# Enigmatisms/AdaPT

Hardware: AMD Instinct MI355X
Metric: Msamples/s (W*H*spp/s), unidirectional MIS path tracing (higher is better)
Workload: dtype f32

## Files before the change

adapt_amd/_lib.py:

```python
from __future__ import annotations

import ctypes as C
import os

_HERE = os.path.dirname(os.path.abspath(__file__))
LIB_PATHS = {"fast": os.environ.get("ADAPT_MI_LIB") or os.path.join(_HERE, "libadapt_mi.so"),
             "exact": os.environ.get("ADAPT_MI_LIB_EXACT") or os.path.join(_HERE, "libadapt_mi_exact.so")}
_variant = "exact" if os.environ.get("APT_EXACT", "0") not in ("", "0") else "fast"
LIB_PATH = LIB_PATHS[_variant]

f32p = C.POINTER(C.c_float)
i32p = C.POINTER(C.c_int32)
u32p = C.POINTER(C.c_uint32)
u8p = C.POINTER(C.c_uint8)
f64p = C.POINTER(C.c_double)
APT_N_KERNELS = 5
KERNEL_NAMES = ("generate", "extend", "shade", "shadow", "finalize")


class AptError(RuntimeError):
    pass


class SceneDesc(C.Structure):
# ... 28 lines not shown
    def as_dict(self):
        d = {k: int(getattr(self, k)) for k in ("n_samples", "n_extend", "n_shade", "n_shadow", "n_shadow_traced", "n_lit", "n_draws", "n_poisoned", "n_track")}
        d["launches"] = dict(zip(KERNEL_NAMES, [int(x) for x in self.launches]))
        d["kernel_ms"] = dict(zip(KERNEL_NAMES, [float(x) for x in self.kernel_ms]))
        d["render_ms"] = float(self.render_ms)
        return d


SYMBOLS = {
    "apt_bvh_build": (C.c_int, [f32p, C.c_int32, i32p, C.c_int32, C.POINTER(C.c_void_p)]),
    "apt_bvh_counts": (C.c_int, [C.c_void_p, i32p, i32p, i32p]),
    "apt_bvh_export": (C.c_int, [C.c_void_p, f32p, i32p]),
    "apt_bvh_wide_counts": (C.c_int, [C.c_void_p, i32p, i32p]),
    "apt_flat_records": (C.c_int, [f32p, C.c_int32, i32p, C.c_int32, i32p, f32p, C.c_int32, f32p, C.c_int32, i32p, i32p]),
    "apt_flat_occluders": (C.c_int, [f32p, C.c_int32, i32p, C.c_int32, i32p, f32p, C.c_int32, C.c_int32, i32p, i32p, C.c_int32, f32p, C.c_int32, i32p, i32p]),
    "apt_bvh_wide_export": (C.c_int, [C.c_void_p, u32p, i32p]),
    "apt_bvh_wide_frame": (C.c_int, [C.c_void_p, f32p, f32p]),
    "apt_bvh_free": (None, [C.c_void_p]),
    "apt_bvh_build_linear": (C.c_int, [f32p, C.c_int32, i32p, i32p, C.c_int32, f32p, f32p, C.POINTER(C.c_void_p)]),
    "apt_linear_bvh_counts": (C.c_int, [C.c_void_p, i32p, i32p]),
    "apt_linear_bvh_export": (C.c_int, [C.c_void_p, f32p, f32p, i32p, i32p]),
    "apt_linear_bvh_free": (None, [C.c_void_p]),
    "apt_scene_create": (C.c_int, [C.POINTER(SceneDesc), C.c_int32, C.POINTER(C.c_void_p)]),
    "apt_scene_destroy": (None, [C.c_void_p]),
    "apt_renderer_create": (C.c_int, [C.c_void_p, C.POINTER(RenderCfg), C.POINTER(C.c_void_p)]),
    "apt_renderer_destroy": (None, [C.c_void_p]),
    "apt_render": (C.c_int, [C.c_void_p, C.c_int32]),
    "apt_synchronize": (C.c_int, [C.c_void_p]),
    "apt_tile_shape": (C.c_int, [C.c_void_p, i32p, i32p]),
    "apt_read_pixels": (C.c_int, [C.c_void_p, f32p]),
# ... 71 lines not shown
```

adapt_amd/csrc/api.hip:

```cpp
#include <hip/hip_runtime.h>
#include <chrono>

#include <algorithm>
#include <cmath>
#include <cstdio>
#include <cstdlib>
#include <cstring>
#include <limits>
#include <memory>
#include <string>
#include <vector>

#include "../../include/adapt_mi.h"
#include "bvh_build.hpp"
#include "shade_stage.hpp"
#include "unit_kernels.hpp"
#include "volumetric.hpp"

#define APT_EXPORT extern "C" __attribute__((visibility("default")))

static thread_local std::string g_err;
static int fail(int code, const std::string& msg) { g_err = msg; return code; }
#define HIP_TRY(expr)                                                                              \
    do {                                                                                           \
// ... 95 lines not shown
template <class... V> static bool put(const char* what, DevBuf& b, const V&... v) {
    const hipError_t e = upload(b, v...);
    if (e != hipSuccess) fail(APT_E_HIP, std::string("upload ") + what + ": " + hipGetErrorString(e));
    return e == hipSuccess;
}

struct apt_bvh { apt::BvhData data; apt::BvhData bin3; apt::WideBvhData wide; };

struct apt_scene {
    int device = 0;
    DevScene dev{};
    int bvh_levels = 0;
    DevBuf nodes, prims, slot_prim, normals, vnormals, precom, prim_obj, prim_class, obj_info, emitter_id, bxdf, src, sweep_recs, sweep_tab;
    DevBuf flat_recs, flat_tab, flat_pairs;
    DevBuf flat_occ, flat_occ_tab;
    bool has_flat = false;
    DevBuf uvs, tex_i, tex_f, atlas[3];
    DevBuf prim_shade;
    DevBuf med;
    DevBuf vol_grid;
    bool has_volume = false;
    bool has_null_surface = false;
    std::vector<int> obj_class;
    std::vector<uint8_t> obj_null;
    float box_min[3] = {1e3f, 1e3f, 1e3f}, box_max[3] = {-1e3f, -1e3f, -1e3f};
    int n_classes = 0;
    int class_def[APT_N_CLASS_DEFS] = {};
    int n_prims = 0, n_objects = 0, n_sources = 0, max_obj_prims = 0;
    int bx_mask = 0, src_mask = 0;
    bool has_aabb = false;
// ... 9 lines not shown
    hipEvent_t fin = nullptr;
    LdsPlan plan{};
    Counters* cnt() const { return counters.as<Counters>(); }
};

struct apt_renderer {
    const apt_scene* scene = nullptr;
    apt_render_cfg cfg{};
    Params par{};
    int n_cols = 0, npix = 0, spp_batch = 1;
    int cnt = 0;
    std::vector<Lane> lanes;
    int n_lanes = 1;
    hipStream_t stream() const { return lanes[0].stream; }
    DevBuf accum, scratch, pix_key;
    Counters host_counters{};
    int grid_small = 0, grid_trace = 0, nq = APT_MAX_NQ;
    const ShadeVariant* shade = nullptr;
    int trace_mode = 0;
    int trace_nt = BLOCK;
    int trace_items = BLOCK;
    int sorted = 0;
    int volumetric = 0;
    int dyn_fetch = 0;
    bool tile_ok = false;
    extend_fn extend = nullptr, fix = nullptr;
    int ovf_levels = 0;
    int v_ncls = 0;
    int vev_single = 0;
    vev_shade_fn vev_all = nullptr;
// ... 288 lines not shown
    const int N = s->n_prims;
    if (N > APT_FLAT_MAX_PRIMS || !s->has_sweep || !d->obj_aabb) return APT_OK;
    std::vector<float> fr, ft; int fc[7];
    if (apt::build_flat(d->prims, N, d->obj_info, s->n_objects, prim_class.data(), fr, ft, fc) != 0) return fail(APT_E_INVALID, "apt_scene_create: flat records: obj_info range outside the primitive array");
    if (!put("flat records", s->flat_recs, fr) || !put("flat records", s->flat_tab, ft) || !put("flat record pairs", s->flat_pairs, apt::flat_pairs(fr, fc))) return APT_E_HIP;
    const bool cull = !(getenv("APT_SHADOW_CULL") && atoi(getenv("APT_SHADOW_CULL")) == 0);
    std::vector<float> pts, op; std::vector<int32_t> off, ot; std::vector<uint8_t> keep;
    apt::emitter_points(d->prims, d->obj_info, s->n_objects, d->src_i, d->src_f, s->n_sources, pts, off);
    if (apt::flat_occluders(d->prims, N, fr, ft, fc, pts.data(), off.data(), s->n_sources, cull, op, ot, keep) != 0) return fail(APT_E_INVALID, "apt_scene_create: flat records: bad record");
    if (!put("occluder lists", s->flat_occ, op) || !put("occluder lists", s->flat_occ_tab, ot)) return APT_E_HIP;
    FlatScene& fl = s->dev.flat;
    fl.stream = s->flat_recs.as<float>(); fl.tab = s->flat_tab.as<float4>(); fl.pairs = s->flat_pairs.as<float>();
    fl.occ_pairs = s->flat_occ.as<float>(); fl.occ_tab = s->flat_occ_tab.as<int>();
    fl.defer_all = getenv("APT_FLAT_DEFER_ALL") ? atoi(getenv("APT_FLAT_DEFER_ALL")) : 0;
    fl.n_quads = fc[0]; fl.n_quads_tie = fc[1]; fl.n_gquads = fc[2]; fl.n_gquads_tie = fc[3]; fl.n_tris = fc[4]; fl.n_tris_tie = fc[5]; fl.n_spheres = fc[6];
    s->has_flat = true;
    if (timer.on) fprintf(stderr, "[scene timing] flat records: %d + %d parallelograms, %d + %d convex quads, %d + %d triangles (plain + coplanar groups), %d spheres of %d primitives\n", fc[0], fc[1], fc[2], fc[3], fc[4], fc[5], fc[6], N);
    if (timer.on) for (int e = 0; e < s->n_sources; e++) fprintf(stderr, "[scene timing] occluders of emitter %d: %d parallelograms, %d convex quads, %d triangles, %d spheres\n", e, ot[8 * (size_t)e + 1], ot[8 * (size_t)e + 2], ot[8 * (size_t)e + 3], ot[8 * (size_t)e + 4]);
    timer.tick("flat records");
    return APT_OK;
}
#endif
static int pack_emitters(const apt_scene_desc* d, apt_scene* s) {
    std::vector<DevSrc> sr((size_t)s->n_sources);
    for (int k = 0; k < s->n_sources; k++) {
        const int32_t* si = d->src_i + 4 * k; const float* sf = d->src_f + 11 * k;
        DevSrc& e = sr[(size_t)k]; memset(&e, 0, sizeof(e));
        e.type = si[0]; e.bool_bits = si[1]; e.obj_ref_id = si[2];
        s->src_mask |= 1 << (e.type & 7);
        e.intensity = mk3(sf[0], sf[1], sf[2]); e.dir = mk3(sf[3], sf[4], sf[5]); e.pos = mk3(sf[6], sf[7], sf[8]); e.inv_area = sf[9]; e.r = sf[10];
// ... 224 lines not shown
        for (int g = 0; g < APT_N_GROUPS; g++) { r->group_fn_[g] = kGroupShade[smi][g]; for (int k = 0; k < APT_GROUP_SLOTS; k++) r->group_cls[g][k] = -1; }
        r->shade_name = "sorted, launched in register-footprint groups:";
        for (int g = 0; g < APT_N_GROUPS; g++) r->group_tr_[g] = kGroupShadeTr[smi][g];
        for (int c = 0; c < sc->n_classes; c++) {
            r->group_cls[kClassGroup[sc->class_def[c]]][kClassSlot[sc->class_def[c]]] = c;
            r->shade_name += std::string(c ? "+" : "") + kClassName[sc->class_def[c]];
        }
    } else {
        r->shade_name = r->shade->name;
        if (p.fused == 2) r->shade_name += " [rays traced in place]";
    }
    if (r->transient) r->shade_name += " [transient]";
    if (r->adaptive) r->shade_name += " [adaptive]";
    r->extend = r->dyn_fetch ? kExtendDyn[r->sorted] : (r->trace_mode == 3 ? kExtendFlatHot[r->sorted] : kExtend[r->trace_mode][r->sorted]);
    r->fix = kFixFlat[r->sorted];
    return APT_OK;
}

static int make_lanes(apt_renderer* r) {
    const apt_scene* sc = r->scene;
    const Params& p = r->par;
    const size_t cap = p.cap, sh_subcap = (size_t)p.subcap * (size_t)(p.S > 0 ? p.S : 1), sh_cap = sh_subcap * (size_t)p.nq;
    const int ncls = r->volumetric ? r->v_ncls : (r->sorted ? sc->n_classes : 0);
    if (cap >= ((size_t)1 << 30) || sh_cap >= ((size_t)1 << 30)) { return fail(APT_E_INVALID, "apt_renderer_create: batch too large (queue capacity must stay below 2^30 slots)"); }
    if (p.fused == 2 && cap >= ((size_t)1 << 28)) { return fail(APT_E_INVALID, "apt_renderer_create: batch too large (rays traced in place address 16-byte slots with 32-bit byte offsets: capacity must stay below 2^28)"); }
    if ((size_t)ncls * cap >= ((size_t)1 << 28)) { return fail(APT_E_INVALID, "apt_renderer_create: batch too large (packed class queues address 16-byte slots with 32-bit byte offsets: classes x capacity must stay below 2^28)"); }
    const bool staged = p.fused != 2, tr_uv = !staged && (sc->dev.has_vn || sc->dev.tex_i != nullptr);
    const bool walk_lists = r->volumetric && sc->has_null_surface;
    const size_t l_planes = (size_t)p.l_planes;
    auto carve = [&](float* base, Queues& q) -> size_t {
// ... 205 lines not shown
    if (!std::isfinite(c.adaptive_threshold)) return fail(APT_E_INVALID, "apt_renderer_create: adaptive_threshold must be finite (> 0: adaptive sampling, <= 0: off)");
    if (c.adaptive_threshold > 0.f) {
        if (c.transient_bins > 0)
            return fail(APT_E_INVALID, "apt_renderer_create: adaptive sampling and transient rendering do not combine (transient_bins must be 0 when adaptive_threshold > 0)");
        if (c.adaptive_min_spp <= 0 || c.adaptive_step <= 0)
            return fail(APT_E_INVALID, "apt_renderer_create: adaptive sampling needs adaptive_min_spp > 0 and adaptive_step > 0");
    }
    HIP_TRY(hipSetDevice(c.device));
    apt_renderer* r = new apt_renderer();
    struct Owner { apt_renderer* r; ~Owner() { if (r) apt_renderer_destroy(r); } } owner{r};
    r->scene = sc; r->cfg = c;
    r->adaptive = c.adaptive_threshold > 0.f ? 1 : 0;
    if (int rc = plan_film(r)) return rc;
    pick_traversal(r);
    if (int rc = pick_shading(r)) return rc;
    if (int rc = make_lanes(r)) return rc;
    if (int rc = make_transient(r)) return rc;
    if (int rc = make_adaptive(r)) return rc;
    if (int rc = plan_lds_and_grids(r)) return rc;
    if (int rc = make_overflow_stacks(r)) return rc;
    for (Lane& ln : r->lanes) HIP_TRY(hipStreamSynchronize(ln.stream));
    owner.r = nullptr;
    *out = r;
    return APT_OK;
}

static int grid_for(size_t n, int cap_blocks, int nq, int nt = BLOCK) {
    size_t b = (n + nt - 1) / nt;
    b = ((b + nq - 1) / nq) * nq;
    if (b < (size_t)nq) b = nq;
// ... 156 lines not shown
    hipEvent_t prev_fin = nullptr;
    const int batch_cap = lane_batch(r, n_spp);
    while (done < n_spp) {
        const int B = (n_spp - done < batch_cap) ? (n_spp - done) : batch_cap;
        Lane& ln = r->lanes[(size_t)(batch % r->n_lanes)];
        hipStream_t st = ln.stream;
        const Queues& q = ln.q;
        Counters* cnt = ln.cnt();
        Params p = r->par; p.cnt_base = r->cnt; p.spp_batch = B;
        const size_t total = (size_t)r->npix * (size_t)B;
        if (int rc = begin_batch(r, ln)) return rc;
#if APT_FAST
        if (p.fused == 2) {
            {
                LaunchTimer t(r, 0, st);
                if (r->adaptive) hipLaunchKernelGGL(k_generate_trace_ad, dim3(grid_for(total, r->grid_small, 1)), dim3(BLOCK), 0, st, sc, p, q, cnt, (const uint8_t*)r->aq.active);
                else hipLaunchKernelGGL(k_generate_trace, dim3(grid_for(total, r->grid_small, 1)), dim3(BLOCK), 0, st, sc, p, q, cnt);
            }
            int cur = 0;
            for (int b = 0; b < p.max_bounce; b++) {
                { LaunchTimer t(r, 2, st); hipLaunchKernelGGL(r->shade->traced, dim3(grid_for(total, r->grid_small, nq)), dim3(BLOCK), 0, st, sc, p, q, cnt, cur, b); }
                cur ^= 1;
            }
            if (p.max_bounce > 0) { LaunchTimer t(r, 3, st, false); hipLaunchKernelGGL(r->fix, dim3(r->grid_fix), dim3(BLOCK), 0, st, sc, p, q, cnt, cur, (const uint32_t*)cnt->n_active[cur], ln.plan); }
        } else
#endif
        {
        {
            LaunchTimer t(r, 0, st);
            if (r->adaptive) hipLaunchKernelGGL(k_generate_ad, dim3(grid_for(total, r->grid_small, 1)), dim3(BLOCK), 0, st, p, q, cnt, (const uint8_t*)r->aq.active);
            else hipLaunchKernelGGL(k_generate, dim3(grid_for(total, r->grid_small, 1)), dim3(BLOCK), 0, st, p, q, cnt);
        }
// ... 438 lines not shown
```

adapt_amd/csrc/bvh_build.hpp:

```cpp
#pragma once
#include <algorithm>
#include <cstdint>
#include <cstdlib>
#include <thread>
#include <vector>

#ifndef APT_NODE_BYTES
#define APT_NODE_BYTES 64u
#endif
#define APT_NODE_DWORDS (APT_NODE_BYTES / 4u)
namespace apt {
inline int host_threads() {
    int t = (int)std::thread::hardware_concurrency();
    t = std::max(1, std::min(t, 32));
    if (const char* e = std::getenv("APT_HOST_THREADS")) t = std::max(1, std::atoi(e));
    return t;
}
template <class F>
void parallel_for(int n, int threads, F f) {
    if (threads <= 1 || n < 2048) { for (int i = 0; i < n; i++) f(i); return; }
    const int t = std::min(threads, (n + 511) / 512);
    std::vector<std::thread> pool;
    pool.reserve((size_t)t);
    for (int k = 0; k < t; k++) {
// ... 30 lines not shown
    std::vector<int32_t> node_info;
    int n_nodes() const { return (int)(node_info.size() / 3); }
    int n_prims() const { return (int)(bvh_info.size() / 2); }
};
int build_linear_bvh(const float* prims, int n_prims, const int32_t* obj_prim_cnt, const int32_t* obj_is_sphere, int n_objects,
                     const float world_min[3], const float world_max[3], LinearBvhData& out);

void planar_rows(const float* tri9, float out12[12]);
int build_flat(const float* prims, int n_prims, const int32_t* obj_info, int n_objects, const int32_t* prim_class,
               std::vector<float>& stream, std::vector<float>& tab, int counts[7]);
std::vector<float> flat_pairs(const std::vector<float>& stream, const int counts[7]);
void emitter_points(const float* prims, const int32_t* obj_info, int n_objects, const int32_t* src_i, const float* src_f, int n_sources,
                    std::vector<float>& pts, std::vector<int32_t>& off);
int flat_occluders(const float* prims, int n_prims, const std::vector<float>& stream, const std::vector<float>& tab, const int counts[7],
                   const float* pts, const int32_t* off, int n_emit, bool cull, std::vector<float>& pairs, std::vector<int32_t>& table, std::vector<uint8_t>& keep);
}
```

adapt_amd/csrc/flat_build.cpp:

```cpp
#include <algorithm>
#include <array>
#include <cmath>
#include <cstring>

#include "bvh_build.hpp"

namespace apt {
namespace {
struct D3 { double x, y, z; };
inline D3 sub(D3 a, D3 b) { return {a.x - b.x, a.y - b.y, a.z - b.z}; }
inline D3 add(D3 a, D3 b) { return {a.x + b.x, a.y + b.y, a.z + b.z}; }
inline D3 cross(D3 a, D3 b) { return {a.y * b.z - a.z * b.y, a.z * b.x - a.x * b.z, a.x * b.y - a.y * b.x}; }
inline double dot(D3 a, D3 b) { return a.x * b.x + a.y * b.y + a.z * b.z; }
inline D3 vtx(const float* prims, int k, int v) { const float* p = prims + 9 * (size_t)k + 3 * v; return {p[0], p[1], p[2]}; }

struct Planar { float P0[3], U[4], V[4], T[4]; int prim_a, prim_b; float map_a[6], map_b[6]; bool ok; int obj; bool tie; float lo[3], hi[3]; float far_edges[6]; };

bool make_rows(D3 p0, D3 e1, D3 e2, Planar& r) {
    const D3 n = cross(e1, e2);
    const double det = dot(n, n);
    if (!(det > 0.0) || !std::isfinite(det)) return false;
    const D3 ru = cross(e2, n), rv = cross(n, e1);
    const D3 U = {ru.x / det, ru.y / det, ru.z / det}, V = {rv.x / det, rv.y / det, rv.z / det};
    const double len = std::sqrt(det);
// ... 305 lines not shown
        }
        std::vector<float> st; int c[7] = {0, 0, 0, 0, 0, 0, 0};
        for (int ri = 0; ri < n_rec; ri++) if (kp[ri]) {
            const Rec& r = recs[(size_t)ri];
            st.insert(st.end(), stream.begin() + (long)r.at, stream.begin() + (long)(r.at + (size_t)kRecordFloats[r.sec]));
            c[2 * r.sec]++;
        }
        int32_t* t = table.data() + 8 * (size_t)e;
        t[0] = (int32_t)pairs.size(); t[1] = c[0]; t[2] = c[2]; t[3] = c[4]; t[4] = c[6];
        std::vector<float> pr = flat_pairs(st, c);
        pairs.insert(pairs.end(), pr.begin(), pr.end());
    }
    if (pairs.empty()) pairs.push_back(0.f);
    return 0;
}
}
```

adapt_amd/csrc/stages.hpp:

```cpp
#pragma once
#include <hip/hip_runtime.h>

#include "rng.hpp"
#include "shading.hpp"
#include "traverse.hpp"
#include "vec.hpp"

struct DevMedium {
    int type;
    float ior;
    f3 u_s, u_a, u_e, par, pdf;
};
struct DevVolume {
    int type, xres, yres, zres;
    f3 albedo, trans, mini, maxi, majorant, pdf;
    f3 inv_r0, inv_r1, inv_r2;
    DevMedium ph;
    const float* grid;
};
struct DevScene {
    DevBvh bvh;
    SweepScene sweep;
    FlatScene flat;
    const float* normals;
// ... 253 lines not shown
    SubLoop s;
    s.q = (int)(blockIdx.x % (uint32_t)nq);
    s.first = (blockIdx.x / (uint32_t)nq) * (uint32_t)nt;
    s.stride = (gridDim.x / (uint32_t)nq) * (uint32_t)nt;
    return s;
}
#ifndef APT_TILE_NT
#define APT_TILE_NT 512
#endif
#ifndef APT_TILE_WAVES
#define APT_TILE_WAVES 6
#endif
#define TRACE_NT(MODE) ((MODE) == 2 ? APT_TILE_NT : BLOCK)

template <bool TRACE, bool ADAPTIVE = false>
APT_D void generate_body(const DevScene* sc, const Params& p, const Queues& q, Counters* cnt, const uint8_t* active = nullptr) {
    const uint32_t total = (uint32_t)p.npix * (uint32_t)p.spp_batch;
    const uint32_t n_waves = (total + 63u) / 64u;
    const uint32_t wave_stride = gridDim.x * (BLOCK / 64);
    uint32_t t_samples = 0, t_draws = 0;
    for (uint32_t w = blockIdx.x * (BLOCK / 64) + threadIdx.x / 64u; w < n_waves; w += wave_stride) {
        const uint32_t idx = w * 64u + lane_id();
        const int sq = (int)(w % (uint32_t)p.nq);
        bool valid = idx < total, alive = false;
        f3 dir = mk3(0.f, 0.f, 1.f);
        uint32_t draws = 0;
        if (valid) {
            uint32_t lp = idx % (uint32_t)p.npix, s = idx / (uint32_t)p.npix;
            int i, j; local_to_global(p, lp, i, j);
            for (int pl = 0; pl < p.l_planes; pl++) stL(q.L, p.cap, (idx << 2) | (uint32_t)pl, splat3(0.f));
            alive = !p.do_crop || (i >= p.sx && i < p.ex && j >= p.sy && j < p.ey);
// ... 21 lines not shown
            }
        }
        uint32_t pos;
        uint32_t* q0_counter = &cnt->n_active[0][sq * CNT_PAD];
        if (TRACE) pos = 0;
        else if (p.do_crop || ADAPTIVE) pos = wave_append(alive, q0_counter);
        else {
            pos = (w / (uint32_t)p.nq) * 64u + lane_id();
            unsigned long long m = __ballot(alive);
            if (lane_id() == 0) atomicAdd(q0_counter, (uint32_t)__popcll(m));
        }
#if APT_FAST
        if (TRACE) {
            const f3 cam_o = mk3(p.cam_t[0], p.cam_t[1], p.cam_t[2]);
            float tr_t = 0.f; int tr_run = -1, tr_idx = -1;
            if (__any(alive)) tr_idx = flat_closest1(sc->flat, cam_o, dir, 1e7f, tr_t, tr_run);
            const bool defer = alive && (tr_run >= 0 || flat_needs_cull(sc->flat, dir));
            HitRec hr; hr.t = 1e7f; hr.prim = -1; hr.u = hr.v = 0.f;
            int hit_cls = 0;
            if (alive && !defer && tr_idx >= 0) flat_resolve(sc->flat, tr_idx, tr_t, cam_o, dir, hr, hit_cls);
            const int ocls = !alive ? -1 : (defer ? q.tr_ncls : (hr.prim >= 0 ? (q.tr_ncls > 1 ? hit_cls : 0) : -1));
            const TrAppend app = tr_append_issue(ocls, q.tr_ncls + 1, &cnt->n_tr[0][0][sq * CNT_PAD], APT_MAX_NQ * CNT_PAD);
            pos = tr_append_pos(app, ocls);
            if (alive) t_samples++;
            if (ocls >= 0) {
                const uint32_t slot = (q.tr_stage_top && ocls == q.tr_ncls) ? (uint32_t)sq * p.subcap + p.subcap - 1u - pos : (uint32_t)ocls * p.cap + (uint32_t)sq * p.subcap + pos, so = slot << 4;
                stq(q.tr[0][0], so, make_float4(cam_o.x, cam_o.y, cam_o.z, hr.t));
                stq(q.tr[0][1], so, make_float4(dir.x, dir.y, dir.z, __uint_as_float(tr_pack(hr.prim, draws, false))));
                stq(q.tr[0][2], so, make_float4(1.f, 1.f, 1.f, __uint_as_float(((idx / (uint32_t)p.npix) << p.pix_bits) | (idx % (uint32_t)p.npix))));
                stq(q.tr[0][3], so, make_float4(0.f, 0.f, 0.f, 1.f));
                if (sc->has_vn || sc->tex_i != nullptr) { float2 uv_; uv_.x = hr.u; uv_.y = hr.v; stq(q.tr_uv[0], slot << 3, uv_); }
// ... 8 lines not shown
            stq(q.id[0], so, ((idx / (uint32_t)p.npix) << p.pix_bits) | (idx % (uint32_t)p.npix));
            stq(q.meta[0], so, pack_meta(draws, 0u, false));
            stq(q.pdf[0], so, 1.f);
            t_samples++;
        }
        t_draws += draws;
    }
    const int sq0 = (int)((blockIdx.x * (BLOCK / 64) + threadIdx.x / 64u) % (uint32_t)p.nq);
    flush_stat(t_samples, &cnt->stats[sq0][ST_SAMPLES]);
    if (TRACE) flush_stat(t_samples, &cnt->stats[sq0][ST_EXTEND]);
    flush_stat(t_draws, &cnt->stats[sq0][ST_DRAWS]);
}
__global__ void __launch_bounds__(BLOCK) k_generate(Params p, Queues q, Counters* cnt) { generate_body<false>(nullptr, p, q, cnt); }
__global__ void __launch_bounds__(BLOCK) k_generate_ad(Params p, Queues q, Counters* cnt, const uint8_t* active) { generate_body<false, true>(nullptr, p, q, cnt, active); }
#if APT_FAST
__global__ void __launch_bounds__(BLOCK) k_generate_trace(DevScene sc, Params p, Queues q, Counters* cnt) { generate_body<true>(&sc, p, q, cnt); }
__global__ void __launch_bounds__(BLOCK) k_generate_trace_ad(DevScene sc, Params p, Queues q, Counters* cnt, const uint8_t* active) { generate_body<true, true>(&sc, p, q, cnt, active); }
#endif

template <int MODE, int SORTED>
__global__ void __launch_bounds__(TRACE_NT(MODE), (MODE == 2 ? APT_TILE_WAVES : 1)) k_extend(DevScene sc, Params p, Queues q, Counters* cnt, int cur, const uint32_t* n_src, LdsPlan plan) {
    __shared__ float s_sweep[MODE == 1 ? APT_SWEEP_LDS_FLOATS(BLOCK) : 1];
    const SubLoop sl = sub_loop(p.nq, TRACE_NT(MODE));
    const uint32_t n = n_src[sl.q * CNT_PAD];
    if (cnt && sl.first == 0 && threadIdx.x == 0) {
        cnt->n_shadow[sl.q * CNT_PAD] = 0; cnt->n_active[cur ^ 1][sl.q * CNT_PAD] = 0;
        for (int w = 0; w < 8; w++) cnt->n_walk[w][sl.q * CNT_PAD] = 0;
        cnt->stats[sl.q][ST_EXTEND] += n;
    }
    const float* ro = q.ray_o[cur]; const float* rd = q.ray_d[cur];
    const uint32_t qbase = (uint32_t)sl.q * p.subcap;
    for (uint32_t base = sl.first; base < n; base += sl.stride) {
// ... 582 lines not shown
```

adapt_amd/csrc/traverse.hpp:

```cpp
#pragma once
#include "vec.hpp"

struct DevBvh {
    const uint4* nodes;
    const float4* prims;
    const int* slot_prim;
    int n_nodes, n_prims;
    float gmin[3], ginv[3], gstep[3];
};
#ifndef APT_FAST_LEAVES
#define APT_FAST_LEAVES APT_FAST
#endif
struct HitRec { float t; int prim; float u, v; };

typedef float v2f __attribute__((ext_vector_type(2)));
APT_D v2f sp2(float s) { v2f r; r.x = s; r.y = s; return r; }
APT_D v2f mk2(float a, float b) { v2f r; r.x = a; r.y = b; return r; }

struct WalkRay { f3 o, d, inv, noo; uint32_t octinv4; };
#ifdef APT_WALK_IEEE_RCP
APT_D float walk_rcp(float d) { return (fabsf(d) < 1e-30f) ? copysignf(1e30f, d) : 1.0f / d; }
#else
APT_D float walk_rcp(float d) { return (fabsf(d) < 1e-30f) ? copysignf(1e30f, d) : __builtin_amdgcn_rcpf(d); }
#endif
// ... 698 lines not shown
        occ = occ || flat_blocks(fminf(fminf(u.x, v.x), w.x) >= 0.f, t.x, lim) || flat_blocks(fminf(fminf(u.y, v.y), w.y) >= 0.f, t.y, lim);
    }
    for (int j = 0; j < ns; j++, at += 8) {
        const v2f r2 = ld2c(at + 6);
        const v2f sx = ld2c(at) - ox, sy = ld2c(at + 2) - oy, sz = ld2c(at + 4) - oz;
        const v2f cn2 = (sx * sx + sy * sy) + sz * sz;
        const v2f proj = (dx * sx + dy * sy) + dz * sz;
        const v2f c2ray = cn2 - proj * proj;
        const v2f disc = r2 - c2ray;
        const float cut0 = sqrtf(disc.x), cut1 = sqrtf(disc.y);
        const float ta = proj.x + ((cn2.x > r2.x + 1e-4f) ? -cut0 : cut0), tb = proj.y + ((cn2.y > r2.y + 1e-4f) ? -cut1 : cut1);
        occ = occ || flat_blocks(c2ray.x < r2.x, ta, lim) || flat_blocks(c2ray.y < r2.y, tb, lim);
    }
    return occ;
}
APT_D int flat_closest1(const FlatScene& fl, f3 o, f3 d, float lim, float& t_out, int& runner) {
    cf_ptr at = (cf_ptr)fl.pairs;
    const v2f ox = sp2(o.x), oy = sp2(o.y), oz = sp2(o.z), dx = sp2(d.x), dy = sp2(d.y), dz = sp2(d.z);
    FlatBest b; b.t = lim; b.idx = -1; b.runner = -1;
    auto solve = [&](cf_ptr r, v2f& t, v2f& u, v2f& v) {
        const v2f sx = ox - ld2c(r), sy = oy - ld2c(r + 2), sz = oz - ld2c(r + 4);
        const v2f ux = ld2c(r + 6), uy = ld2c(r + 8), uz = ld2c(r + 10);
        const v2f vx = ld2c(r + 12), vy = ld2c(r + 14), vz = ld2c(r + 16);
        const v2f tx = ld2c(r + 18), ty = ld2c(r + 20), tz = ld2c(r + 22);
        const v2f t_o = fma2(tx, sx, fma2(ty, sy, tz * sz));
        const v2f t_d = fma2(tx, dx, fma2(ty, dy, tz * dz));
        v2f inv; inv.x = __builtin_amdgcn_rcpf(t_d.x); inv.y = __builtin_amdgcn_rcpf(t_d.y);
        t = -t_o * inv;
        const v2f px = fma2(t, dx, sx), py = fma2(t, dy, sy), pz = fma2(t, dz, sz);
        u = fma2(ux, px, fma2(uy, py, uz * pz));
        v = fma2(vx, px, fma2(vy, py, vz * pz));
    };
    int idx = 0;
    {
        const int n = fl.n_quads + fl.n_quads_tie, n_plain = fl.n_quads >> 1;
        int j = 0;
        for (; j < n_plain; j++, idx += 2, at += 24) {
            v2f t, u, v; solve(at, t, u, v);
            const v2f a = u - sp2(0.5f), c = v - sp2(0.5f);
            b = flat_candidate<false>(b, fmaxf(fabsf(a.x), fabsf(c.x)) <= 0.5f, t.x, idx);
            b = flat_candidate<false>(b, fmaxf(fabsf(a.y), fabsf(c.y)) <= 0.5f, t.y, idx + 1);
        }
        for (; 2 * j < n; j++, idx += 2, at += 24) {
            v2f t, u, v; solve(at, t, u, v);
            const v2f a = u - sp2(0.5f), c = v - sp2(0.5f);
            b = flat_candidate<true>(b, fmaxf(fabsf(a.x), fabsf(c.x)) <= 0.5f, t.x, idx);
            b = flat_candidate<true>(b, 2 * j + 1 < n && fmaxf(fabsf(a.y), fabsf(c.y)) <= 0.5f, t.y, idx + 1);
        }
        idx = n;
    }
    {
        const int n = fl.n_gquads + fl.n_gquads_tie, n_plain = fl.n_gquads >> 1, first = idx;
        int j = 0;
        for (; j < n_plain; j++, idx += 2, at += 36) {
            v2f t, u, v; solve(at, t, u, v);
            const v2f e1 = fma2(ld2c(at + 24), u, fma2(ld2c(at + 26), v, ld2c(at + 28))), e2 = fma2(ld2c(at + 30), u, fma2(ld2c(at + 32), v, ld2c(at + 34)));
            b = flat_candidate<false>(b, fminf(fminf(u.x, v.x), fminf(e1.x, e2.x)) >= 0.f, t.x, idx);
            b = flat_candidate<false>(b, fminf(fminf(u.y, v.y), fminf(e1.y, e2.y)) >= 0.f, t.y, idx + 1);
        }
        for (; 2 * j < n; j++, idx += 2, at += 36) {
            v2f t, u, v; solve(at, t, u, v);
            const v2f e1 = fma2(ld2c(at + 24), u, fma2(ld2c(at + 26), v, ld2c(at + 28))), e2 = fma2(ld2c(at + 30), u, fma2(ld2c(at + 32), v, ld2c(at + 34)));
            b = flat_candidate<true>(b, fminf(fminf(u.x, v.x), fminf(e1.x, e2.x)) >= 0.f, t.x, idx);
            b = flat_candidate<true>(b, 2 * j + 1 < n && fminf(fminf(u.y, v.y), fminf(e1.y, e2.y)) >= 0.f, t.y, idx + 1);
        }
        idx = first + n;
    }
    {
        const int n = fl.n_tris + fl.n_tris_tie, n_plain = fl.n_tris >> 1, first = idx;
        int j = 0;
        for (; j < n_plain; j++, idx += 2, at += 24) {
            v2f t, u, v; solve(at, t, u, v);
            const v2f w = (sp2(1.0f) - u) - v;
            b = flat_candidate<false>(b, fminf(fminf(u.x, v.x), w.x) >= 0.f, t.x, idx);
            b = flat_candidate<false>(b, fminf(fminf(u.y, v.y), w.y) >= 0.f, t.y, idx + 1);
        }
        for (; 2 * j < n; j++, idx += 2, at += 24) {
            v2f t, u, v; solve(at, t, u, v);
            const v2f w = (sp2(1.0f) - u) - v;
            b = flat_candidate<true>(b, fminf(fminf(u.x, v.x), w.x) >= 0.f, t.x, idx);
            b = flat_candidate<true>(b, 2 * j + 1 < n && fminf(fminf(u.y, v.y), w.y) >= 0.f, t.y, idx + 1);
        }
        idx = first + n;
    }
    for (int j = 0; 2 * j < fl.n_spheres; j++, idx += 2, at += 8) {
        const v2f r2 = ld2c(at + 6);
        const v2f sx = ld2c(at) - ox, sy = ld2c(at + 2) - oy, sz = ld2c(at + 4) - oz;
        const v2f cn2 = (sx * sx + sy * sy) + sz * sz;
        const v2f proj = (dx * sx + dy * sy) + dz * sz;
        const v2f c2ray = cn2 - proj * proj;
        const v2f disc = r2 - c2ray;
        const float cut0 = sqrtf(disc.x), cut1 = sqrtf(disc.y);
        const float ta = proj.x + ((cn2.x > r2.x + 1e-4f) ? -cut0 : cut0), tb = proj.y + ((cn2.y > r2.y + 1e-4f) ? -cut1 : cut1);
        b = flat_candidate<false>(b, c2ray.x < r2.x, ta, idx);
        b = flat_candidate<false>(b, 2 * j + 1 < fl.n_spheres && c2ray.y < r2.y, tb, idx + 1);
    }
    if ((fl.n_quads_tie | fl.n_gquads_tie | fl.n_tris_tie) != 0) {
        const int a0 = fl.n_quads, a1 = a0 + fl.n_quads_tie, b0 = a1 + fl.n_gquads, b1 = b0 + fl.n_gquads_tie, c0 = b1 + fl.n_tris, c1 = c0 + fl.n_tris_tie;
        const bool tie = (b.idx >= a0 && b.idx < a1) || (b.idx >= b0 && b.idx < b1) || (b.idx >= c0 && b.idx < c1);
        b.runner = tie ? b.runner : -1;
// ... 6 lines not shown
```

include/adapt_mi.h:

```cpp
#ifndef ADAPT_MI_H
#define ADAPT_MI_H

#include <stdint.h>

#ifdef __cplusplus
extern "C" {
#endif

#define APT_OK            0
#define APT_E_INVALID    -1
#define APT_E_NO_DEVICE  -2
#define APT_E_HIP        -3
#define APT_E_NOMEM      -4
#define APT_E_STATE      -5

typedef struct apt_bvh apt_bvh;
typedef struct apt_scene apt_scene;
typedef struct apt_renderer apt_renderer;

typedef struct apt_scene_desc {
    int32_t n_prims, n_objects, n_sources, has_vertex_normal;
    const float*   prims;
    const float*   normals;
    const float*   v_normals;
// ... 59 lines not shown
int apt_bvh_build(const float* prims , int32_t n_prims,
                  const int32_t* obj_info , int32_t n_objects, apt_bvh** out);
int apt_bvh_counts(const apt_bvh*, int32_t* n_nodes, int32_t* n_leaf_prims, int32_t* max_depth);
int apt_bvh_export(const apt_bvh*, float* nodes, int32_t* prim_order);
int apt_bvh_wide_counts(const apt_bvh*, int32_t* n_nodes, int32_t* n_levels);
int apt_bvh_wide_export(const apt_bvh*, uint32_t* nodes , int32_t* prim_order );
int apt_bvh_wide_frame(const apt_bvh*, float gmin[3], float gstep[3]);
void apt_bvh_free(apt_bvh*);

int apt_flat_records(const float* prims , int32_t n_prims, const int32_t* obj_info , int32_t n_objects,
                     int32_t counts[7], float* stream, int32_t stream_cap, float* tab, int32_t tab_cap, int32_t* n_stream, int32_t* n_tab);
int apt_flat_occluders(const float* prims , int32_t n_prims, const int32_t* obj_info , int32_t n_objects,
                       const int32_t* src_i, const float* src_f, int32_t n_sources, int32_t cull, int32_t* table, int32_t* keep, int32_t keep_cap,
                       float* pairs, int32_t pairs_cap, int32_t* n_records, int32_t* n_pairs);

typedef struct apt_linear_bvh apt_linear_bvh;
int apt_bvh_build_linear(const float* prims , int32_t n_prims, const int32_t* obj_prim_cnt, const int32_t* obj_is_sphere,
                         int32_t n_objects, const float* world_min , const float* world_max , apt_linear_bvh** out);
int apt_linear_bvh_counts(const apt_linear_bvh*, int32_t* n_nodes, int32_t* n_prims);
int apt_linear_bvh_export(const apt_linear_bvh*, float* bvh_minmax, float* node_minmax, int32_t* bvh_info, int32_t* node_info);
void apt_linear_bvh_free(apt_linear_bvh*);

int apt_scene_create(const apt_scene_desc* desc, int32_t device, apt_scene** out);
void apt_scene_destroy(apt_scene*);
int apt_renderer_create(const apt_scene*, const apt_render_cfg* cfg, apt_renderer** out);
void apt_renderer_destroy(apt_renderer*);

int apt_render(apt_renderer*, int32_t n_spp);
int apt_synchronize(apt_renderer*);
int apt_tile_shape(const apt_renderer*, int32_t* n_cols, int32_t* height);
// ... 37 lines not shown
```

Before: 5405.

## Cull flat primitive pairs per 64-pixel camera strip in primary-ray tracing

At renderer creation the host builds, for each block of 64 film pixels, a frustum from the block's pixel bounds and tests every flat-scene primitive pair against it with conservative floating-point margins, producing a 64-bit mask of pairs that could be visible. The fused generate+trace kernel loads the mask for its wave from scalar memory and skips pair intersection tests whose bit is clear. This cuts primary-ray intersection work in the flat-scene path, at the cost of host-side precomputation, an extra device buffer and per-pair branch checks. Correctness depends on the conservative margins covering every pixel's possible hits.

```diff
diff --git a/adapt_amd/_lib.py b/adapt_amd/_lib.py
--- a/adapt_amd/_lib.py
+++ b/adapt_amd/_lib.py
@@ -66,6 +66,7 @@
     "apt_bvh_wide_counts": (C.c_int, [C.c_void_p, i32p, i32p]),
     "apt_flat_records": (C.c_int, [f32p, C.c_int32, i32p, C.c_int32, i32p, f32p, C.c_int32, f32p, C.c_int32, i32p, i32p]),
     "apt_flat_occluders": (C.c_int, [f32p, C.c_int32, i32p, C.c_int32, i32p, f32p, C.c_int32, C.c_int32, i32p, i32p, C.c_int32, f32p, C.c_int32, i32p, i32p]),
+    "apt_camera_strips": (C.c_int, [f32p, C.c_int32, i32p, C.c_int32, C.POINTER(RenderCfg), C.c_int32, C.POINTER(C.c_uint64), C.c_int32, i32p, i32p]),
     "apt_bvh_wide_export": (C.c_int, [C.c_void_p, u32p, i32p]),
     "apt_bvh_wide_frame": (C.c_int, [C.c_void_p, f32p, f32p]),
     "apt_bvh_free": (None, [C.c_void_p]),
diff --git a/adapt_amd/csrc/api.hip b/adapt_amd/csrc/api.hip
--- a/adapt_amd/csrc/api.hip
+++ b/adapt_amd/csrc/api.hip
@@ -133,6 +133,7 @@
     DevBuf nodes, prims, slot_prim, normals, vnormals, precom, prim_obj, prim_class, obj_info, emitter_id, bxdf, src, sweep_recs, sweep_tab;
     DevBuf flat_recs, flat_tab, flat_pairs;
     DevBuf flat_occ, flat_occ_tab;
+    std::vector<float> h_prims, h_flat_recs, h_flat_tab; int h_flat_counts[7] = {0, 0, 0, 0, 0, 0, 0};
     bool has_flat = false;
     DevBuf uvs, tex_i, tex_f, atlas[3];
     DevBuf prim_shade;
@@ -172,6 +173,7 @@
     int n_lanes = 1;
     hipStream_t stream() const { return lanes[0].stream; }
     DevBuf accum, scratch, pix_key;
+    DevBuf cam_strips;
     Counters host_counters{};
     int grid_small = 0, grid_trace = 0, nq = APT_MAX_NQ;
     const ShadeVariant* shade = nullptr;
@@ -490,6 +492,7 @@
     fl.occ_pairs = s->flat_occ.as<float>(); fl.occ_tab = s->flat_occ_tab.as<int>();
     fl.defer_all = getenv("APT_FLAT_DEFER_ALL") ? atoi(getenv("APT_FLAT_DEFER_ALL")) : 0;
     fl.n_quads = fc[0]; fl.n_quads_tie = fc[1]; fl.n_gquads = fc[2]; fl.n_gquads_tie = fc[3]; fl.n_tris = fc[4]; fl.n_tris_tie = fc[5]; fl.n_spheres = fc[6];
+    s->h_prims.assign(d->prims, d->prims + 9 * (size_t)N); s->h_flat_recs = fr; s->h_flat_tab = ft; memcpy(s->h_flat_counts, fc, sizeof(fc));
     s->has_flat = true;
     if (timer.on) fprintf(stderr, "[scene timing] flat records: %d + %d parallelograms, %d + %d convex quads, %d + %d triangles (plain + coplanar groups), %d spheres of %d primitives\n", fc[0], fc[1], fc[2], fc[3], fc[4], fc[5], fc[6], N);
     if (timer.on) for (int e = 0; e < s->n_sources; e++) fprintf(stderr, "[scene timing] occluders of emitter %d: %d parallelograms, %d convex quads, %d triangles, %d spheres\n", e, ot[8 * (size_t)e + 1], ot[8 * (size_t)e + 2], ot[8 * (size_t)e + 3], ot[8 * (size_t)e + 4]);
@@ -744,6 +747,42 @@
     if (r->adaptive) r->shade_name += " [adaptive]";
     r->extend = r->dyn_fetch ? kExtendDyn[r->sorted] : (r->trace_mode == 3 ? kExtendFlatHot[r->sorted] : kExtend[r->trace_mode][r->sorted]);
     r->fix = kFixFlat[r->sorted];
+    return APT_OK;
+}
+
+static apt::CamFilm cam_film(const apt_render_cfg& c) {
+    apt::CamFilm cf;
+    memcpy(cf.cam_r, c.cam_r, sizeof(cf.cam_r)); memcpy(cf.cam_t, c.cam_t, sizeof(cf.cam_t));
+    cf.inv_focal = c.inv_focal; cf.half_w = c.half_w; cf.half_h = c.half_h;
+    cf.width = c.width; cf.height = c.height; cf.n_cols = owned_columns(c); cf.band_width = c.band_width; cf.rank = c.rank; cf.world = c.world_size;
+    return cf;
+}
+static int make_camera_strips(apt_renderer* r) {
+    if (r->par.fused != 2) return APT_OK;
+    const apt_scene* sc = r->scene;
+    const bool cull = !(getenv("APT_CAMERA_CULL") && atoi(getenv("APT_CAMERA_CULL")) == 0);
+    std::vector<uint64_t> masks;
+    if (apt::camera_strips(sc->h_prims.data(), sc->n_prims, sc->h_flat_recs, sc->h_flat_tab, sc->h_flat_counts, cam_film(r->cfg), cull, masks) != 0)
+        return fail(APT_E_INVALID, "apt_renderer_create: camera strip lists: bad record or film");
+    hipError_t e = upload(r->cam_strips, masks);
+    if (e != hipSuccess) return fail(APT_E_HIP, std::string("upload camera strip lists: ") + hipGetErrorString(e));
+    return APT_OK;
+}
+
+APT_EXPORT int apt_camera_strips(const float* prims, int32_t n_prims, const int32_t* obj_info, int32_t n_objects, const apt_render_cfg* cfg, int32_t cull,
+                                 uint64_t* masks, int32_t masks_cap, int32_t* n_strips, int32_t* n_pairs) {
+    if (!prims || !obj_info || !cfg || n_prims <= 0 || n_objects <= 0 || !n_strips || !n_pairs) return fail(APT_E_INVALID, "apt_camera_strips: bad argument");
+    apt_render_cfg c = *cfg;
+    if (c.world_size <= 0) { c.world_size = 1; c.rank = 0; }
+    if (c.band_width <= 0) c.band_width = c.width;
+    if (c.width <= 0 || c.height <= 0 || c.rank < 0 || c.rank >= c.world_size || owned_columns(c) <= 0) return fail(APT_E_INVALID, "apt_camera_strips: bad film or rank");
+    std::vector<float> st, tb; int cn[7];
+    if (apt::build_flat(prims, n_prims, obj_info, n_objects, nullptr, st, tb, cn) != 0) return fail(APT_E_INVALID, "apt_camera_strips: obj_info range outside the primitive array");
+    std::vector<uint64_t> m;
+    if (apt::camera_strips(prims, n_prims, st, tb, cn, cam_film(c), cull != 0, m) != 0) return fail(APT_E_INVALID, "apt_camera_strips: bad record or film");
+    *n_strips = (int32_t)m.size();
+    *n_pairs = (cn[0] + cn[1] + 1) / 2 + (cn[2] + cn[3] + 1) / 2 + (cn[4] + cn[5] + 1) / 2 + (cn[6] + 1) / 2;
+    if (masks) { if (masks_cap < (int32_t)m.size()) return fail(APT_E_INVALID, "apt_camera_strips: masks buffer too small"); memcpy(masks, m.data(), m.size() * 8); }
     return APT_OK;
 }
 
@@ -979,6 +1018,7 @@
     if (int rc = plan_film(r)) return rc;
     pick_traversal(r);
     if (int rc = pick_shading(r)) return rc;
+    if (int rc = make_camera_strips(r)) return rc;
     if (int rc = make_lanes(r)) return rc;
     if (int rc = make_transient(r)) return rc;
     if (int rc = make_adaptive(r)) return rc;
@@ -1165,8 +1205,9 @@
         if (p.fused == 2) {
             {
                 LaunchTimer t(r, 0, st);
-                if (r->adaptive) hipLaunchKernelGGL(k_generate_trace_ad, dim3(grid_for(total, r->grid_small, 1)), dim3(BLOCK), 0, st, sc, p, q, cnt, (const uint8_t*)r->aq.active);
-                else hipLaunchKernelGGL(k_generate_trace, dim3(grid_for(total, r->grid_small, 1)), dim3(BLOCK), 0, st, sc, p, q, cnt);
+                const unsigned long long* strips = r->cam_strips.as<unsigned long long>();
+                if (r->adaptive) hipLaunchKernelGGL(k_generate_trace_ad, dim3(grid_for(total, r->grid_small, 1)), dim3(BLOCK), 0, st, sc, p, q, cnt, (const uint8_t*)r->aq.active, strips);
+                else hipLaunchKernelGGL(k_generate_trace, dim3(grid_for(total, r->grid_small, 1)), dim3(BLOCK), 0, st, sc, p, q, cnt, strips);
             }
             int cur = 0;
             for (int b = 0; b < p.max_bounce; b++) {
diff --git a/adapt_amd/csrc/bvh_build.hpp b/adapt_amd/csrc/bvh_build.hpp
--- a/adapt_amd/csrc/bvh_build.hpp
+++ b/adapt_amd/csrc/bvh_build.hpp
@@ -68,4 +68,10 @@
                     std::vector<float>& pts, std::vector<int32_t>& off);
 int flat_occluders(const float* prims, int n_prims, const std::vector<float>& stream, const std::vector<float>& tab, const int counts[7],
                    const float* pts, const int32_t* off, int n_emit, bool cull, std::vector<float>& pairs, std::vector<int32_t>& table, std::vector<uint8_t>& keep);
+#ifndef APT_FLAT_MAX_PRIMS
+#define APT_FLAT_MAX_PRIMS 96
+#endif
+struct CamFilm { float cam_r[9], cam_t[3], inv_focal, half_w, half_h; int width, height, n_cols, band_width, rank, world; };
+int camera_strips(const float* prims, int n_prims, const std::vector<float>& stream, const std::vector<float>& tab, const int counts[7],
+                  const CamFilm& cf, bool cull, std::vector<uint64_t>& masks);
 }
diff --git a/adapt_amd/csrc/flat_build.cpp b/adapt_amd/csrc/flat_build.cpp
--- a/adapt_amd/csrc/flat_build.cpp
+++ b/adapt_amd/csrc/flat_build.cpp
@@ -343,4 +343,102 @@
     if (pairs.empty()) pairs.push_back(0.f);
     return 0;
 }
-}
+
+int camera_strips(const float* prims, int n_prims, const std::vector<float>& stream, const std::vector<float>& tab, const int counts[7],
+                  const CamFilm& cf, bool cull, std::vector<uint64_t>& masks) {
+    static_assert((APT_FLAT_MAX_PRIMS + 4) / 2 <= 64, "a strip's pair list is one 64-bit word (four sections, each with at most one odd tail)");
+    const double u = std::ldexp(1.0, -24);
+    const int nsec[4] = {counts[0] + counts[1], counts[2] + counts[3], counts[4] + counts[5], counts[6]};
+    const int n_pairs = (nsec[0] + 1) / 2 + (nsec[1] + 1) / 2 + (nsec[2] + 1) / 2 + (nsec[3] + 1) / 2;
+    const int npix = cf.n_cols * cf.height, n_blocks = (npix + 63) / 64;
+    if (npix <= 0 || cf.height <= 0 || cf.band_width <= 0 || cf.world <= 0) return -1;
+    const uint64_t all = ~(uint64_t)0;
+    masks.assign((size_t)n_blocks, all);
+    if (!cull || n_pairs > 64) return 0;
+    const D3 cam = {cf.cam_t[0], cf.cam_t[1], cf.cam_t[2]};
+    struct Rec { int pair; std::vector<D3> vs; double margin; };
+    std::vector<Rec> recs;
+    double lo[3] = {cam.x, cam.y, cam.z}, hi[3] = {cam.x, cam.y, cam.z};
+    {
+        size_t at = 0; int pair0 = 0;
+        for (int sec = 0, r = 0; sec < 4; pair0 += (nsec[sec] + 1) / 2, sec++) for (int j = 0; j < nsec[sec]; j++, r++, at += (size_t)kRecordFloats[sec]) {
+            int32_t ids[2]; memcpy(ids, tab.data() + 28 * (size_t)r + 8, 8);
+            if (ids[0] < 0 || ids[0] >= n_prims || ids[1] >= n_prims) return -1;
+            Rec rc; rc.pair = pair0 + j / 2; rc.margin = 0.0;
+            if (sec < 3) { for (int k : {ids[0], ids[1]}) if (k >= 0) for (int v = 0; v < 3; v++) rc.vs.push_back(vtx(prims, k, v)); }
+            else {
+                const float* c = prims + 9 * (size_t)ids[0];
+                const D3 dc = sub({c[0], c[1], c[2]}, cam);
+                const double D2 = dot(dc, dc), rr = std::sqrt((double)c[3] * (double)c[3] * (1.0 + 4.0 * u) + 1.1e-4 + 32.0 * u * D2);
+                for (int k = 0; k < 8; k++) rc.vs.push_back({c[0] + ((k & 1) ? rr : -rr), c[1] + ((k & 2) ? rr : -rr), c[2] + ((k & 4) ? rr : -rr)});
+                rc.margin = 16.0 * 6.0 * u * (std::sqrt(D2) + rr);
+            }
+            for (const D3& p : rc.vs) { const double c[3] = {p.x, p.y, p.z}; for (int a = 0; a < 3; a++) { lo[a] = std::min(lo[a], c[a]); hi[a] = std::max(hi[a], c[a]); } }
+            recs.push_back(rc);
+        }
+    }
+    const D3 ext = {hi[0] - lo[0], hi[1] - lo[1], hi[2] - lo[2]};
+    const double L = std::sqrt(dot(ext, ext));
+    auto absdot = [](D3 a, D3 b) { return std::fabs(a.x) * b.x + std::fabs(a.y) * b.y + std::fabs(a.z) * b.z; };
+    {
+        size_t at = 0;
+        for (int sec = 0, r = 0; sec < 3; sec++) for (int j = 0; j < nsec[sec]; j++, r++, at += (size_t)kRecordFloats[sec]) {
+            const float* p = stream.data() + at;
+            const D3 U = {p[3], p[4], p[5]}, V = {p[6], p[7], p[8]}, T = {p[9], p[10], p[11]};
+            if (dot(T, T) == 0.0) continue;
+            std::vector<std::array<double, 3>> edges = {{1, 0, 0}, {0, 1, 0}};
+            if (sec == 0) { edges.push_back({1, 0, 0.5}); edges.push_back({0, 1, 0.5}); }
+            if (sec == 2) edges.push_back({1, 1, 1});
+            if (sec == 1) for (int e = 0; e < 2; e++) edges.push_back({p[12 + 3 * e], p[13 + 3 * e], p[14 + 3 * e]});
+            double ovs = 0.0;
+            for (const auto& g : edges) {
+                const D3 grad = add({g[0] * U.x, g[0] * U.y, g[0] * U.z}, {g[1] * V.x, g[1] * V.y, g[1] * V.z});
+                const double gl = std::sqrt(dot(grad, grad));
+                if (!(gl > 0.0)) return -1;
+                ovs = std::max(ovs, (5.0 * u * (std::fabs(g[0]) * absdot(U, ext) + std::fabs(g[1]) * absdot(V, ext)) + 3.0 * u * (std::fabs(g[0]) + std::fabs(g[1]) + std::fabs(g[2]))) / gl);
+            }
+            recs[(size_t)r].margin = 16.0 * ((7.0 * u * absdot(T, ext) + 6.0 * u * L) / std::sqrt(dot(T, T)) + ovs);
+        }
+    }
+    const double widen = 64.0 * u * ((double)cf.width + (double)cf.height + 1.0 / std::fabs((double)cf.inv_focal));
+    auto world = [&](double x, double y) -> D3 {
+        const float* R = cf.cam_r;
+        return {R[0] * x + R[1] * y + R[2], R[3] * x + R[4] * y + R[5], R[6] * x + R[7] * y + R[8]};
+    };
+    for (int b = 0; b < n_blocks; b++) {
+        int i0 = 1 << 30, i1 = -(1 << 30), j0 = 1 << 30, j1 = -(1 << 30);
+        for (int lp = 64 * b; lp < std::min(npix, 64 * b + 64); lp++) {
+            const int lc = lp / cf.height, j = lp % cf.height, i = (lc / cf.band_width * cf.world + cf.rank) * cf.band_width + lc % cf.band_width;
+            i0 = std::min(i0, i); i1 = std::max(i1, i); j0 = std::min(j0, j); j1 = std::max(j1, j);
+        }
+        const double f = cf.inv_focal;
+        double xa = ((double)cf.half_w - i1 - widen) * f, xb = ((double)cf.half_w + 1.0 - i0 + widen) * f;
+        double ya = ((double)j0 - cf.half_h - 1.0 - widen) * f, yb = ((double)j1 - cf.half_h + widen) * f;
+        if (xa > xb) std::swap(xa, xb);
+        if (ya > yb) std::swap(ya, yb);
+        const D3 c[4] = {world(xa, ya), world(xb, ya), world(xb, yb), world(xa, yb)}, mid = world(0.5 * (xa + xb), 0.5 * (ya + yb));
+        D3 n[4];
+        bool ok = true;
+        for (int k = 0; k < 4; k++) {
+            D3 m = cross(c[k], c[(k + 1) & 3]);
+            const double len = std::sqrt(dot(m, m));
+            if (!(len > 0.0) || !std::isfinite(len)) { ok = false; break; }
+            if (dot(m, mid) < 0.0) m = {-m.x, -m.y, -m.z};
+            n[k] = {m.x / len, m.y / len, m.z / len};
+        }
+        if (!ok) continue;
+        uint64_t m = 0;
+        for (const Rec& r : recs) {
+            bool out = false;
+            for (int k = 0; k < 4 && !out; k++) {
+                double top = -1e300;
+                for (const D3& p : r.vs) top = std::max(top, dot(n[k], sub(p, cam)));
+                out = top < -r.margin;
+            }
+            if (!out) m |= (uint64_t)1 << r.pair;
+        }
+        masks[(size_t)b] = m;
+    }
+    return 0;
+}
+}
diff --git a/adapt_amd/csrc/stages.hpp b/adapt_amd/csrc/stages.hpp
--- a/adapt_amd/csrc/stages.hpp
+++ b/adapt_amd/csrc/stages.hpp
@@ -291,7 +291,7 @@
 #define TRACE_NT(MODE) ((MODE) == 2 ? APT_TILE_NT : BLOCK)
 
 template <bool TRACE, bool ADAPTIVE = false>
-APT_D void generate_body(const DevScene* sc, const Params& p, const Queues& q, Counters* cnt, const uint8_t* active = nullptr) {
+APT_D void generate_body(const DevScene* sc, const Params& p, const Queues& q, Counters* cnt, const uint8_t* active = nullptr, const unsigned long long* strips = nullptr) {
     const uint32_t total = (uint32_t)p.npix * (uint32_t)p.spp_batch;
     const uint32_t n_waves = (total + 63u) / 64u;
     const uint32_t wave_stride = gridDim.x * (BLOCK / 64);
@@ -343,7 +343,12 @@
         if (TRACE) {
             const f3 cam_o = mk3(p.cam_t[0], p.cam_t[1], p.cam_t[2]);
             float tr_t = 0.f; int tr_run = -1, tr_idx = -1;
-            if (__any(alive)) tr_idx = flat_closest1(sc->flat, cam_o, dir, 1e7f, tr_t, tr_run);
+            if (__any(alive)) {
+                typedef const __attribute__((address_space(4))) unsigned long long* strip_ptr;
+                const uint32_t lp0 = (uint32_t)__builtin_amdgcn_readfirstlane((int)((w * 64u) % (uint32_t)p.npix)), lp1 = lp0 + 63u, last = (uint32_t)p.npix - 1u;
+                const unsigned long long mask = ((strip_ptr)strips)[lp0 >> 6] | ((strip_ptr)strips)[(lp1 < last ? lp1 : last) >> 6] | ((strip_ptr)strips)[lp1 > last ? 0u : (lp0 >> 6)];
+                tr_idx = flat_closest1<true>(sc->flat, cam_o, dir, 1e7f, tr_t, tr_run, mask);
+            }
             const bool defer = alive && (tr_run >= 0 || flat_needs_cull(sc->flat, dir));
             HitRec hr; hr.t = 1e7f; hr.prim = -1; hr.u = hr.v = 0.f;
             int hit_cls = 0;
@@ -382,8 +387,8 @@
 __global__ void __launch_bounds__(BLOCK) k_generate(Params p, Queues q, Counters* cnt) { generate_body<false>(nullptr, p, q, cnt); }
 __global__ void __launch_bounds__(BLOCK) k_generate_ad(Params p, Queues q, Counters* cnt, const uint8_t* active) { generate_body<false, true>(nullptr, p, q, cnt, active); }
 #if APT_FAST
-__global__ void __launch_bounds__(BLOCK) k_generate_trace(DevScene sc, Params p, Queues q, Counters* cnt) { generate_body<true>(&sc, p, q, cnt); }
-__global__ void __launch_bounds__(BLOCK) k_generate_trace_ad(DevScene sc, Params p, Queues q, Counters* cnt, const uint8_t* active) { generate_body<true, true>(&sc, p, q, cnt, active); }
+__global__ void __launch_bounds__(BLOCK) k_generate_trace(DevScene sc, Params p, Queues q, Counters* cnt, const unsigned long long* strips) { generate_body<true>(&sc, p, q, cnt, nullptr, strips); }
+__global__ void __launch_bounds__(BLOCK) k_generate_trace_ad(DevScene sc, Params p, Queues q, Counters* cnt, const uint8_t* active, const unsigned long long* strips) { generate_body<true, true>(&sc, p, q, cnt, active, strips); }
 #endif
 
 template <int MODE, int SORTED>
diff --git a/adapt_amd/csrc/traverse.hpp b/adapt_amd/csrc/traverse.hpp
--- a/adapt_amd/csrc/traverse.hpp
+++ b/adapt_amd/csrc/traverse.hpp
@@ -736,7 +736,8 @@
     }
     return occ;
 }
-APT_D int flat_closest1(const FlatScene& fl, f3 o, f3 d, float lim, float& t_out, int& runner) {
+template <bool MASKED = false>
+APT_D int flat_closest1(const FlatScene& fl, f3 o, f3 d, float lim, float& t_out, int& runner, unsigned long long mask = ~0ull) {
     cf_ptr at = (cf_ptr)fl.pairs;
     const v2f ox = sp2(o.x), oy = sp2(o.y), oz = sp2(o.z), dx = sp2(d.x), dy = sp2(d.y), dz = sp2(d.z);
     FlatBest b; b.t = lim; b.idx = -1; b.runner = -1;
@@ -754,16 +755,20 @@
         v = fma2(vx, px, fma2(vy, py, vz * pz));
     };
     int idx = 0;
+    int k = 0;
+    auto skip = [&](int pair) { return MASKED && ((mask >> (pair & 63)) & 1ull) == 0ull; };
     {
         const int n = fl.n_quads + fl.n_quads_tie, n_plain = fl.n_quads >> 1;
         int j = 0;
-        for (; j < n_plain; j++, idx += 2, at += 24) {
+        for (; j < n_plain; j++, idx += 2, at += 24, k++) {
+            if (skip(k)) continue;
             v2f t, u, v; solve(at, t, u, v);
             const v2f a = u - sp2(0.5f), c = v - sp2(0.5f);
             b = flat_candidate<false>(b, fmaxf(fabsf(a.x), fabsf(c.x)) <= 0.5f, t.x, idx);
             b = flat_candidate<false>(b, fmaxf(fabsf(a.y), fabsf(c.y)) <= 0.5f, t.y, idx + 1);
         }
-        for (; 2 * j < n; j++, idx += 2, at += 24) {
+        for (; 2 * j < n; j++, idx += 2, at += 24, k++) {
+            if (skip(k)) continue;
             v2f t, u, v; solve(at, t, u, v);
             const v2f a = u - sp2(0.5f), c = v - sp2(0.5f);
             b = flat_candidate<true>(b, fmaxf(fabsf(a.x), fabsf(c.x)) <= 0.5f, t.x, idx);
@@ -774,13 +779,15 @@
     {
         const int n = fl.n_gquads + fl.n_gquads_tie, n_plain = fl.n_gquads >> 1, first = idx;
         int j = 0;
-        for (; j < n_plain; j++, idx += 2, at += 36) {
+        for (; j < n_plain; j++, idx += 2, at += 36, k++) {
+            if (skip(k)) continue;
             v2f t, u, v; solve(at, t, u, v);
             const v2f e1 = fma2(ld2c(at + 24), u, fma2(ld2c(at + 26), v, ld2c(at + 28))), e2 = fma2(ld2c(at + 30), u, fma2(ld2c(at + 32), v, ld2c(at + 34)));
             b = flat_candidate<false>(b, fminf(fminf(u.x, v.x), fminf(e1.x, e2.x)) >= 0.f, t.x, idx);
             b = flat_candidate<false>(b, fminf(fminf(u.y, v.y), fminf(e1.y, e2.y)) >= 0.f, t.y, idx + 1);
         }
-        for (; 2 * j < n; j++, idx += 2, at += 36) {
+        for (; 2 * j < n; j++, idx += 2, at += 36, k++) {
+            if (skip(k)) continue;
             v2f t, u, v; solve(at, t, u, v);
             const v2f e1 = fma2(ld2c(at + 24), u, fma2(ld2c(at + 26), v, ld2c(at + 28))), e2 = fma2(ld2c(at + 30), u, fma2(ld2c(at + 32), v, ld2c(at + 34)));
             b = flat_candidate<true>(b, fminf(fminf(u.x, v.x), fminf(e1.x, e2.x)) >= 0.f, t.x, idx);
@@ -791,13 +798,15 @@
     {
         const int n = fl.n_tris + fl.n_tris_tie, n_plain = fl.n_tris >> 1, first = idx;
         int j = 0;
-        for (; j < n_plain; j++, idx += 2, at += 24) {
+        for (; j < n_plain; j++, idx += 2, at += 24, k++) {
+            if (skip(k)) continue;
             v2f t, u, v; solve(at, t, u, v);
             const v2f w = (sp2(1.0f) - u) - v;
             b = flat_candidate<false>(b, fminf(fminf(u.x, v.x), w.x) >= 0.f, t.x, idx);
             b = flat_candidate<false>(b, fminf(fminf(u.y, v.y), w.y) >= 0.f, t.y, idx + 1);
         }
-        for (; 2 * j < n; j++, idx += 2, at += 24) {
+        for (; 2 * j < n; j++, idx += 2, at += 24, k++) {
+            if (skip(k)) continue;
             v2f t, u, v; solve(at, t, u, v);
             const v2f w = (sp2(1.0f) - u) - v;
             b = flat_candidate<true>(b, fminf(fminf(u.x, v.x), w.x) >= 0.f, t.x, idx);
@@ -805,7 +814,8 @@
         }
         idx = first + n;
     }
-    for (int j = 0; 2 * j < fl.n_spheres; j++, idx += 2, at += 8) {
+    for (int j = 0; 2 * j < fl.n_spheres; j++, idx += 2, at += 8, k++) {
+        if (skip(k)) continue;
         const v2f r2 = ld2c(at + 6);
         const v2f sx = ld2c(at) - ox, sy = ld2c(at + 2) - oy, sz = ld2c(at + 4) - oz;
         const v2f cn2 = (sx * sx + sy * sy) + sz * sz;
diff --git a/include/adapt_mi.h b/include/adapt_mi.h
--- a/include/adapt_mi.h
+++ b/include/adapt_mi.h
@@ -97,6 +97,9 @@
                        const int32_t* src_i, const float* src_f, int32_t n_sources, int32_t cull, int32_t* table, int32_t* keep, int32_t keep_cap,
                        float* pairs, int32_t pairs_cap, int32_t* n_records, int32_t* n_pairs);
 
+int apt_camera_strips(const float* prims , int32_t n_prims, const int32_t* obj_info , int32_t n_objects,
+                      const apt_render_cfg* cfg, int32_t cull, uint64_t* masks, int32_t masks_cap, int32_t* n_strips, int32_t* n_pairs);
+
 typedef struct apt_linear_bvh apt_linear_bvh;
 int apt_bvh_build_linear(const float* prims , int32_t n_prims, const int32_t* obj_prim_cnt, const int32_t* obj_is_sphere,
                          int32_t n_objects, const float* world_min , const float* world_max , apt_linear_bvh** out);
```

After: 5519, median of 6. 1.02x the previous value.
